# hjmkt/wrenc

Hardware: AMD Instinct MI355X
Metric: all-intra encode fps at fixed QP (CTU RD search + final pass); bit-exactness vs the CPU oracle is checked in `parity` (higher is better)
Workload: dtype u8/i16/i32 (+i64 trellis costs, f32 RD cost)

## Files before the change

wrenc_amd/csrc/dev_quant.h:

```cpp
#pragma once

namespace wrenc {

__device__ __forceinline__ long long ldq_at(Ctx c, int bits) {
    return bits < 256 ? (long long)SHT.ldq[bits] : c.k->ldq[bits];
}
__device__ __forceinline__ long long lv_at(Ctx c, int a) {
    return a < 256 ? (long long)SHT.lv[a] : c.k->lv[a];
}
template <int CTRL>
__device__ __forceinline__ int dpp_quad(int v) {
    return __builtin_amdgcn_mov_dpp(v, CTRL, 0xF, 0xF, true);
}

struct DecMasks {
    uint32_t m01, m23;
};
__device__ __forceinline__ DecMasks dec_masks(const uint16_t* dec16, int p) {
    const uint2 v = *(const uint2*)(dec16 + (p >> 4) * 4);
    DecMasks m;
    m.m01 = v.x;
    m.m23 = v.y;
    return m;
}
__device__ __forceinline__ int dec_nib(DecMasks m, int p) {
    const int k = p & 15;
    const uint32_t t01 = m.m01 >> k, t23 = m.m23 >> k;
    return (int)((t01 & 1u) | ((t01 >> 15) & 2u) | ((t23 & 1u) << 2) | ((t23 >> 13) & 8u));
}

constexpr int kMapId = 0x03020100;
__device__ __forceinline__ int compose_map(int g2, int g1) {
    return (int)__builtin_amdgcn_perm(0u, (uint32_t)g2, (uint32_t)g1);
}
__device__ __forceinline__ int position_map(int tc, int qd, bool dcn, int nib) {
    int pv = 0;
    if (tc != 0) {
        const int b0 = (qd >> 1) & 1;
        const int b1 = dcn ? b0 : (((qd + 1) >> 1) & 1);
        pv = nib ^ (b0 ? 3 : 0) ^ (b1 ? 12 : 0);
    }
    const unsigned x = (unsigned)(pv ^ 10);
    return (int)(0x01010000u + (((x * 0x00204081u) & 0x01010101u) << 1));
}

constexpr int kNoBranch = 1 << 27;

__device__ __forceinline__ int ldq_fast(const Ctx& c, int idx) {
    int v = SHT.ldq[min(idx, 255)];
    if (__ballot(idx > 255) != 0ULL) {
        if (idx > 255) v = (int)c.k->ldq[idx];
    }
    return v;
}

__device__ __forceinline__ int quotient(const CONST_AS DevConst* k, int tc, int sh, int off) {
    int S = (int)((unsigned)tc << sh) - off;
    if (tc < 0) S = -S;
    return tc == 0 ? 0 : (int)(__umulhi((unsigned)S, k->div_magic) >> k->div_shift);
}

__device__ __forceinline__ void chunk_entry(const Ctx& c, int* en, int tc, int qd, bool dcn, bool tzp, int sh, int off,
                                            int lsc, int ldq1, int* par0_out, int* par1_out, int* adj_out,
                                            int* ovf) {
    const bool nz = tc != 0;
    int c0d[2], c1d[2], par[2];
#pragma unroll
    for (int d = 0; d < 2; ++d) {
        const int a0 = (qd + (dcn ? 0 : d)) >> 1;
        const int a1 = a0 + 1;
        int q0 = (a0 > 0 || dcn) ? 2 * a0 - d : 0;
        int q1 = 2 * a1 - d;
        if (tc < 0) {
            q0 = -q0;
            q1 = -q1;
        }
        const int d0 = abs(tc - ((M24(q0, lsc) + off) >> sh));
        const int d1 = abs(tc - ((M24(q1, lsc) + off) >> sh));
        if (nz && a1 + 1 >= 1024) *ovf = 1;
        const int l0 = ldq_fast(c, min(a0 + 1, 1023)), l1 = ldq_fast(c, min(a1 + 1, 1023));
        c0d[d] = nz ? 128 * d0 + l0 : ldq1;
        c1d[d] = nz ? 128 * d1 + l1 : kNoBranch;
        par[d] = nz ? (a0 & 1) : 0;
    }
    const int a00 = qd >> 1;
    const bool zero0 = !nz || a00 == 0;
    const int c0tz = nz ? (a00 == 0 ? c0d[0] - ldq1 : c0d[0]) : 0;
    const int c0s0 = tzp ? c0tz : c0d[0];
    const int p0 = par[0], p1 = par[1];
    en[0] = 2 * (p0 ? c1d[0] : c0s0) + p0;
    en[1] = 2 * (p0 ? c0s0 : c1d[0]) + 1 - p0;
    en[2] = 2 * (p0 ? c1d[0] : c0d[0]) + p0;
    en[3] = 2 * (p0 ? c0d[0] : c1d[0]) + 1 - p0;
    en[4] = 2 * (p1 ? c1d[1] : c0d[1]) + p1;
    en[5] = 2 * (p1 ? c0d[1] : c1d[1]) + 1 - p1;
    *par0_out = p0;
    *par1_out = p1;
    *adj_out = (tzp && zero0) ? 1 : 0;
}

__device__ __forceinline__ int lv_fast(const Ctx& c, int a) {
    int v = SHT.lv[min(a, 255)];
    if (__ballot(a > 255) != 0ULL) {
        if (a > 255) v = (int)c.k->lv[a];
    }
    return v;
}

__device__ __forceinline__ int emit_level(const Ctx& c, int tc, int qd, bool dcn, int nib, int p, int j, int& state,
                                          unsigned& zmask, long long& sum_nz, int& fnz, int& ovf) {
    const int dl = state > 1 ? 1 : 0;
    const bool nz = tc != 0;
    const int a = nz ? ((qd + (dcn ? 0 : dl)) >> 1) + ((nib >> state) & 1) : 0;
    int q = (nz && (a > 0 || dcn)) ? 2 * a - dl : 0;
    if (tc < 0) q = -q;
    const int qc = abs(q);
    const bool zero = qc == 0;
    zmask |= (zero ? 1u : 0u) << j;
    const int aw = (qc + dl) >> 1;
    if (!zero && aw >= 1024) ovf = 1;
    const int lv = lv_fast(c, min(aw, 1023));
    sum_nz += zero ? 0 : lv;
    fnz = zero ? fnz : min(fnz, p);
    state = (0x7D28 >> (2 * (2 * state + (a & 1)))) & 3;
    return q;
}

__device__ __forceinline__ unsigned shift_in_less(unsigned bits, int kb, int ka) {
    return __builtin_amdgcn_alignbit(bits, (unsigned)(kb - ka), 31);
}

constexpr int kAlphaInf = 1 << 28;
struct HeadK {
    int ldq1, ldq2, ldq3;
    int dp1, dp2, dp3, dn1, dn2, dn3;
};
__device__ __forceinline__ HeadK head_consts(int sh, int off, int lsc) {
    HeadK h;
    h.ldq1 = uni(SHT.ldq[1]);
    h.ldq2 = uni(SHT.ldq[2]);
    h.ldq3 = uni(SHT.ldq[3]);
    h.dp1 = (lsc + off) >> sh;
    h.dp2 = (2 * lsc + off) >> sh;
    h.dp3 = (3 * lsc + off) >> sh;
    h.dn1 = (-lsc + off) >> sh;
    h.dn2 = (-2 * lsc + off) >> sh;
    h.dn3 = (-3 * lsc + off) >> sh;
    return h;
}
__device__ __forceinline__ int head_alpha(int tc, int qd, bool dcn, const HeadK& h, bool* bad) {
    const bool neg = tc < 0;
    const int d1 = abs(tc - (neg ? h.dn1 : h.dp1));
    const int d2 = abs(tc - (neg ? h.dn2 : h.dp2));
    const int d3 = abs(tc - (neg ? h.dn3 : h.dp3));
    const int d1o = abs(tc - (neg ? h.dp1 : h.dn1));
    const int c0tz = 128 * abs(tc);
    const int c0d0 = c0tz + h.ldq1;
    const int c1d0 = 128 * d2 + h.ldq2;
    const int c0d1 = dcn ? 128 * d1o + h.ldq1 : (qd ? 128 * d1 + h.ldq2 : c0d0);
    const int c1d1 = (qd && !dcn) ? 128 * d3 + h.ldq3 : 128 * d1 + h.ldq2;
    int alpha = c1d0 - c0tz;
    int beta = min(min(c0d0, c0d1), c1d1) - c0tz;
    if (tc == 0) {
        alpha = kAlphaInf;
        beta = h.ldq1;
    }
    *bad = qd >= 2 || alpha < 0 || beta < 0 || h.ldq1 < 0;
    return min(alpha, kAlphaInf);
}
struct HeadT {
    int tn, cnt, tnd, cntd, tnq, cntq;
};
__device__ __forceinline__ HeadT head_ranges(const CONST_AS DevConst* k, int lg) {
    const CONST_AS int32_t* r = k->head_rng[lg - 2];
    HeadT t;
    t.tn = r[0];
    t.cnt = r[1];
    t.tnd = r[2];
    t.cntd = r[3];
    t.tnq = r[4];
    t.cntq = r[5];
    return t;
}
__device__ __forceinline__ bool head_bad(int tc, bool dcn, const HeadT& t) {
    return (unsigned)(tc + (dcn ? t.tnd : t.tn)) >= (unsigned)(dcn ? t.cntd : t.cnt);
}
__device__ __forceinline__ bool head_sig(int tc, const HeadT& t) { return (unsigned)(tc + t.tnq) >= (unsigned)t.cntq; }
__device__ __forceinline__ int head_alpha1(int tc, const HeadK& h) {
    const int d2 = abs(tc - (tc < 0 ? h.dn2 : h.dp2));
    return tc == 0 ? kAlphaInf : min(128 * d2 + h.ldq2 - 128 * abs(tc), kAlphaInf);
}
__device__ __forceinline__ void head_batch(int tc, int p, int P, bool valid, const HeadK& h, const HeadT& t, bool& open, int& arun, int& sb) {
    if (!open) return;
    const int alpha = head_alpha1(tc, h);
    const unsigned long long B = __ballot(valid && head_bad(tc, p == P - 1, t));
    if (B == 0ULL) {
        if (valid) arun = min(arun, alpha);
    } else {
        const int fb = (int)__builtin_ctzll(B);
        sb = (p - LANE + fb) >> 4;
        if (valid && LANE < (fb & ~15)) arun = min(arun, alpha);
        open = false;
    }
}
__device__ __forceinline__ int head_sb(bool open, int sb, int nsb) { return open ? nsb : sb; }
__device__ __forceinline__ bool head_test(int C, int st, int amin) {
    const int c0 = dpp_quad<0x00>(C);
    int m = st == 0 ? 0x7FFFFFFF : C;
    m = min(m, dpp_quad<0xB1>(m));
    m = min(m, dpp_quad<0x4E>(m));
    return (m - c0) + 2 * amin >= 0;
}

template <int LG>
__device__ __forceinline__ void solo_gather(int blk, int16_t* tcs, const HeadK& hk, const HeadT& ht, int& nzl, int& first, bool& open,
                                            int& arun, int& sb) {
    constexpr int P = 1 << (2 * LG), NB = (P + 63) / 64, G = 4;
    const int lane = LANE;
    const int row = lane >> 4;
    const int in4 = blk * P + scan_nib_offset(LG, scan_nib(lane & 15));
#pragma unroll
    for (int g = 0; g < NB; g += G) {
        int tcb[G];
#pragma unroll
        for (int t = 0; t < G; ++t) {
            if (g + t >= NB) continue;
            const int p = 64 * (g + t) + lane;
            tcb[t] = p < P ? (int)SH.r1[scan_word_origin(scan_batch_word(LG, g + t), row) + in4] : 0;
        }
#pragma unroll
        for (int t = 0; t < G; ++t) {
            if (g + t >= NB) continue;
            const int p0 = 64 * (g + t), p = p0 + lane;
            const bool valid = p < P;
            const int tc = tcb[t];
            nzl |= tc;
            if (valid) tcs[blk * P + p] = (int16_t)tc;
            if (first == P) {
                const unsigned long long sig = __ballot(head_sig(tc, ht));
                if (sig != 0ULL) first = p0 + (int)__builtin_ctzll(sig);
            }
            head_batch(tc, p, P, valid, hk, ht, open, arun, sb);
        }
    }
}

__device__ __forceinline__ long long quantize_solo(Ctx c, int lg, int nb, int* overflow, bool* any_level) {
    c = uni(c);
    lg = uni(lg);
    nb = uni(nb);
    const CONST_AS DevConst* k = c.k;
    const int n = 1 << lg;
    const int P = n * n;
    const int lgP = 2 * lg;
    const int sh = 8 + lg - 5 + 1;
    const int off = (1 << sh) >> 1;
    const int lsc = k->lsc;
    int16_t* tcs = (int16_t*)SH.r2;
    int32_t* cc = (int32_t*)SH.r1;
    uint16_t* dec16 = (uint16_t*)SH.decw;
    PROF_MARK(q0_);
    *any_level = false;
#ifdef WRENC_EXP_SKIP_QUANT
    for (int i = LANE; i < (nb * P) / 8; i += 64) *(uint4*)&SH.r1[8 * i] = make_uint4(0u, 0u, 0u, 0u);
    WSYNC();
    return 0;
#endif
    const HeadK hk = head_consts(sh, off, lsc);
    const HeadT ht = head_ranges(k, lg);
    const int nsb = P >> 4;
    int istar0 = P, istar1 = P, sbs0 = nsb - 1, sbs1 = nsb - 1, amin0 = kAlphaInf, amin1 = kAlphaInf;
    int nzl = 0;
#pragma unroll 1
    for (int blk = 0; blk < nb; ++blk) {
        int first = P, arun = kAlphaInf, sb = nsb - 1;
        bool open = true;
        switch (lg) {
        case 2: solo_gather<2>(blk, tcs, hk, ht, nzl, first, open, arun, sb); break;
        case 3: solo_gather<3>(blk, tcs, hk, ht, nzl, first, open, arun, sb); break;
        case 4: solo_gather<4>(blk, tcs, hk, ht, nzl, first, open, arun, sb); break;
        default: solo_gather<5>(blk, tcs, hk, ht, nzl, first, open, arun, sb); break;
        }
        sb = head_sb(open, sb, nsb);
        if (sb > 0 && sb < nsb) arun = wave_min_i32(arun);
        if (blk) {
            istar1 = first;
            sbs1 = sb;
            amin1 = arun;
        } else {
            istar0 = first;
            sbs0 = sb;
            amin0 = arun;
        }
    }
    if (__ballot(nzl != 0) == 0ULL) return 0;
    WSYNC();
    if (sbs0 == nsb && (nb == 1 || sbs1 == nsb)) {
        for (int i = LANE; i < (nb * P) / 8; i += 64) *(uint4*)&SH.r1[8 * i] = make_uint4(0u, 0u, 0u, 0u);
        WSYNC();
        PROF_MARK(qz_);
        PROF_ADD2(PH_QPRE, q0_, qz_);
        return 0;
    }
    if (LANE < sbs0) *(uint2*)(dec16 + LANE * 4) = make_uint2(0u, 0u);
    if (nb == 2 && LANE < sbs1) *(uint2*)(dec16 + (P >> 2) + LANE * 4) = make_uint2(0u, 0u);
    PROF_MARK(q1_);
    PROF_ADD2(PH_QPRE, q0_, q1_);
    const int ldq1 = hk.ldq1;
    const int st = LANE & 3;
    const int CH = min(P, nb == 2 ? 32 : 64);
    const int quad = LANE >> 2;
    const bool walker = quad < nb;
    const int wblk = walker ? quad : 0;
    const int32_t* wcc = (const int32_t*)SH.r1 + wblk * CH * 6;
    const int cls = st == 0 ? 0 : (st == 1 ? 1 : 2);
    uint16_t* wdec = dec16 + wblk * (P >> 2);
    int wsb = wblk ? sbs1 : sbs0;
    const int wamin = wblk ? amin1 : amin0;
    int lowest = nb == 2 ? min(sbs0, sbs1) : sbs0;
    int C = 0;
    int ovf = 0;
    for (int base = P - CH; base >= 0 && base + CH > 16 * lowest; base -= CH) {
        PROF_MARK(qb0_);
        WSYNC();
        {
            const bool mine = LANE < nb * CH;
            const int blk = LANE >= CH ? 1 : 0;
            const int i = LANE - blk * CH;
            const int p = base + i;
            int par0 = 0, par1 = 0, adj = 0;
            if (mine) {
                const int tc = tcs[blk * P + p];
                chunk_entry(c, cc + LANE * 6, tc, quotient(k, tc, sh, off), p == P - 1, p <= (blk ? istar1 : istar0),
                            sh, off, lsc, ldq1, &par0, &par1, &adj, &ovf);
            }
            const unsigned long long b0 = __ballot(mine && par0), b1 = __ballot(mine && par1), ba = __ballot(mine && adj);
            if (mine && (LANE & 15) == 0) {
                uint16_t* pm = SH.q_pm[blk][i >> 4];
                pm[0] = (uint16_t)(b0 >> LANE);
                pm[1] = (uint16_t)(b1 >> LANE);
                pm[2] = (uint16_t)((ba >> (LANE + 15)) & 1);
            }
        }
        WSYNC();
        PROF_MARK(qb1_);
        if (walker) {
            for (int g16 = CH - 16; g16 >= 0; g16 -= 16) {
                const int sb = (base + g16) >> 4;
                if (sb < lowest) break;
                const uint16_t* pm = SH.q_pm[wblk][g16 >> 4];
                const unsigned parmask = pm[st > 1 ? 1 : 0];
                const bool adj = st == 0 && pm[2] != 0;
                int2 cur[16];
#pragma unroll
                for (int kk = 0; kk < 16; ++kk) cur[kk] = *(const int2*)&wcc[(g16 + kk) * 6 + 2 * cls];
                unsigned bits = 0;
#pragma unroll
                for (int kk = 15; kk >= 0; --kk) {
                    const int2 e = cur[kk];
                    const int KA = e.x + dpp_quad<0xD8>(C);
                    const int KB = e.y + dpp_quad<0x72>(C);
                    C = min(KA, KB) & ~1;
                    bits = shift_in_less(bits, KB, KA);
                    if (kk == 15) {
                        const bool choseB = KB < KA;
                        const bool pick1 = choseB != (((parmask >> 15) & 1) != 0);
                        if (!pick1 && adj) C -= 2 * ldq1;
                    }
                }
                bits ^= parmask;
                int m = min(C, dpp_quad<0xB1>(C));
                m = min(m, dpp_quad<0x4E>(m));
                C -= m;
                wdec[sb * 4 + st] = (uint16_t)bits;
                const bool proven = head_test(C, st, wamin);
                if (sb == wsb && sb > 0 && !proven) wsb = 0;
                lowest = __builtin_amdgcn_readlane(wsb, 0);
                if (nb == 2) lowest = min(lowest, __builtin_amdgcn_readlane(wsb, 4));
            }
        }
        lowest = __builtin_amdgcn_readlane(wsb, 0);
        if (nb == 2) lowest = min(lowest, __builtin_amdgcn_readlane(wsb, 4));
        PROF_MARK(qb3_);
        PROF_ADD2(PH_QB_PRE, qb0_, qb1_);
        PROF_ADD2(PH_QB_WALK, qb1_, qb3_);
    }
    WSYNC();
    PROF_MARK(q2_);
    PROF_ADD2(PH_QBACK, q1_, q2_);
    const int start0 = 16 * __builtin_amdgcn_readlane(wsb, 0), start1 = nb == 2 ? 16 * __builtin_amdgcn_readlane(wsb, 4) : 0;
    for (int i = LANE; i < (nb * P) / 8; i += 64) *(uint4*)&SH.r1[8 * i] = make_uint4(0u, 0u, 0u, 0u);
    WSYNC();
    const int half = nb == 2 ? 32 : 64;
    const int blk = nb == 2 ? (LANE >> 5) : 0;
    const int lane_in = LANE & (half - 1);
    const int start = blk ? start1 : start0;
    int per = 1;
    while (per * half < P - start) per *= 2;
    const int p0 = start + lane_in * per;
    const bool act = p0 < P;
    const int16_t* btcs = tcs + blk * P;
    const uint16_t* bdec = dec16 + blk * (P >> 2);
    int fmap = kMapId;
    const DecMasks dm = dec_masks(bdec, act ? p0 : 0);
    const int org = blk * P + scan_sb_origin(lg, act ? p0 >> 4 : 0);
    if (act) {
        for (int j = 0; j < per; ++j) {
            const int p = p0 + j;
            const int tc = btcs[p];
            fmap = compose_map(position_map(tc, quotient(k, tc, sh, off), p == P - 1, dec_nib(dm, p)), fmap);
        }
    }
    int pre = fmap;
    pre = compose_map(pre, __builtin_amdgcn_update_dpp(kMapId, pre, 0x111, 0xF, 0xF, false));
    pre = compose_map(pre, __builtin_amdgcn_update_dpp(kMapId, pre, 0x112, 0xF, 0xF, false));
    pre = compose_map(pre, __builtin_amdgcn_update_dpp(kMapId, pre, 0x114, 0xF, 0xF, false));
    pre = compose_map(pre, __builtin_amdgcn_update_dpp(kMapId, pre, 0x118, 0xF, 0xF, false));
    pre = compose_map(pre, __builtin_amdgcn_update_dpp(kMapId, pre, 0x142, 0xA, 0xF, false));
    if (nb == 1) pre = compose_map(pre, __builtin_amdgcn_update_dpp(kMapId, pre, 0x143, 0xC, 0xF, false));
    int entry = __builtin_amdgcn_update_dpp(0, pre, 0x138, 0xF, 0xF, false) & 3;
    if (lane_in == 0) entry = 0;
    long long sum_nz = 0;
    unsigned zmask = 0;
    int fnz = P;
    if (act) {
        int state = entry;
        unsigned long long nibs = scan_nibs_from(p0 & 15);
        for (int j = 0; j < per; ++j, nibs >>= 4) {
            const int p = p0 + j;
            const int tc = btcs[p];
            SH.r1[org + scan_nib_offset(lg, (int)nibs & 15)] = (int16_t)emit_level(c, tc, quotient(k, tc, sh, off), p == P - 1, dec_nib(dm, p), p, j,
                                                                                  state, zmask, sum_nz, fnz, ovf);
        }
    }
    const int pf = group_min_i32(fnz, half);
    if (act)
        sum_nz += (long long)__popc(zmask >> min(max(pf - p0 + 1, 0), 16)) * SHT.lv[0];
    *any_level = __ballot(pf < P) != 0ULL;
    const long long sum = wave_sum_i64(sum_nz);
    if (__ballot(ovf != 0) != 0ULL) *overflow = 1;
    WSYNC();
    PROF_MARK(q3_);
    PROF_ADD2(PH_QTRACE, q2_, q3_);
    return sum;
}

__device__ __forceinline__ int quantize_p16_reg(Ctx c, int nb, int coef, int* overflow, long long lvl[4], int* any_mask) {
    c = uni(c);
    nb = uni(nb);
    const int lane = lane_fresh();
    const CONST_AS DevConst* k = c.k;
    constexpr int P = 16, lg = 2;
    constexpr int sh = 8 + lg - 5 + 1;
    constexpr int off = (1 << sh) >> 1;
    const int lsc = k->lsc;
    int32_t* cc = (int32_t*)SH.r1;
    PROF_MARK(q0_);
    const int blk = lane >> 4, p = lane & 15;
    const bool mine = blk < nb;
#ifdef WRENC_EXP_SKIP_QUANT
    lvl[0] = lvl[1] = lvl[2] = lvl[3] = 0;
    *any_mask = 0;
    WSYNC();
    return 0;
#endif
    const HeadT ht = head_ranges(k, 2);
    const int at = 16 * blk + scan_nib(p);
    int tc = __builtin_amdgcn_ds_bpermute(4 * at, coef);
    if (!mine) tc = 0;
    const int istar = row_min_i32(head_sig(tc, ht) ? p : P);
    const unsigned long long nzb = __ballot(tc != 0);
    lvl[0] = lvl[1] = lvl[2] = lvl[3] = 0;
    *any_mask = 0;
    if (nzb == 0ULL) return 0;
    if (__ballot(mine && head_bad(tc, p == P - 1, ht)) == 0ULL) return 0;
    PROF_MARK(q1_);
    PROF_ADD2(PH_QPRE, q0_, q1_);
    WSYNC();
    const int qd = quotient(k, tc, sh, off);
    const int ldq1 = (int)ldq_at(c, 1);
    int ovf = 0;
    {
        int par0 = 0, par1 = 0, adj = 0;
        if (mine) chunk_entry(c, cc + lane * 6, tc, qd, p == P - 1, p <= istar, sh, off, lsc, ldq1, &par0, &par1, &adj, &ovf);
        const unsigned long long b0 = __ballot(mine && par0), b1 = __ballot(mine && par1), ba = __ballot(mine && adj);
        if (mine && p == 0) {
            uint16_t* pm = SH.q_pm[0][blk];
            pm[0] = (uint16_t)(b0 >> lane);
            pm[1] = (uint16_t)(b1 >> lane);
            pm[2] = (uint16_t)((ba >> (lane + 15)) & 1);
        }
    }
    WSYNC();
    PROF_MARK(qb1_);
    uint16_t* dec16 = (uint16_t*)SH.decw;
    {
        const int st = lane & 3, quad = lane >> 2;
        if (quad < nb) {
            const int cls = st == 0 ? 0 : (st == 1 ? 1 : 2);
            const int32_t* wcc = cc + quad * P * 6;
            const uint16_t* pm = SH.q_pm[0][quad];
            const unsigned parmask = pm[st > 1 ? 1 : 0];
            const bool adj = st == 0 && pm[2] != 0;
            int2 cur[16];
#pragma unroll
            for (int kk = 0; kk < 16; ++kk) cur[kk] = *(const int2*)&wcc[kk * 6 + 2 * cls];
            unsigned bits = 0;
            int C = 0;
#pragma unroll
            for (int kk = 15; kk >= 0; --kk) {
                const int2 e = cur[kk];
                const int KA = e.x + dpp_quad<0xD8>(C);
                const int KB = e.y + dpp_quad<0x72>(C);
                C = min(KA, KB) & ~1;
                bits = shift_in_less(bits, KB, KA);
                if (kk == 15) {
                    const bool choseB = KB < KA;
                    const bool pick1 = choseB != (((parmask >> 15) & 1) != 0);
                    if (!pick1 && adj) C -= 2 * ldq1;
                }
            }
            bits ^= parmask;
            dec16[quad * 4 + st] = (uint16_t)bits;
        }
    }
    WSYNC();
    PROF_MARK(q2_);
    PROF_ADD2(PH_QBACK, q1_, q2_);
    PROF_ADD2(PH_QB_WALK, qb1_, q2_);
    const DecMasks dm = dec_masks(dec16 + blk * 4, 0);
    const int nib = dec_nib(dm, p);
    int pre = mine ? position_map(tc, qd, p == P - 1, nib) : kMapId;
    pre = compose_map(pre, __builtin_amdgcn_update_dpp(kMapId, pre, 0x111, 0xF, 0xF, false));
    pre = compose_map(pre, __builtin_amdgcn_update_dpp(kMapId, pre, 0x112, 0xF, 0xF, false));
    pre = compose_map(pre, __builtin_amdgcn_update_dpp(kMapId, pre, 0x114, 0xF, 0xF, false));
    pre = compose_map(pre, __builtin_amdgcn_update_dpp(kMapId, pre, 0x118, 0xF, 0xF, false));
    int entry = __builtin_amdgcn_update_dpp(0, pre, 0x111, 0xF, 0xF, false) & 3;
    if (p == 0) entry = 0;
    long long sum_nz = 0;
    unsigned zmask = 0;
    int fnz = P;
    int level = 0;
    if (mine) {
        int state = entry;
        level = (int16_t)emit_level(c, tc, qd, p == P - 1, nib, p, 0, state, zmask, sum_nz, fnz, ovf);
    }
    level = __builtin_amdgcn_ds_permute(4 * at, level);
    const int pf = row_min_i32(fnz);
    if (mine && (zmask & 1u) && p > pf) sum_nz += SHT.lv[0];
    {
        const long long hi = sum_nz >> 24;
        const int ra = row_sum_i32((int)(sum_nz & 0xFFFFFF)), rb = row_sum_i32((int)(hi & 0xFFFFFF)), rc = row_sum_i32((int)(hi >> 24));
#pragma unroll
        for (int b = 0; b < 4; ++b) {
            const long long a0 = (long long)(unsigned)__builtin_amdgcn_readlane(ra, 16 * b);
            const long long a1 = (long long)(unsigned)__builtin_amdgcn_readlane(rb, 16 * b);
            const long long a2 = (long long)__builtin_amdgcn_readlane(rc, 16 * b);
            lvl[b] = a0 + ((a1 + (a2 << 24)) << 24);
            if (__builtin_amdgcn_readlane(pf, 16 * b) < P) *any_mask |= 1 << b;
        }
    }
    if (__ballot(ovf != 0) != 0ULL) *overflow = 1;
    WSYNC();
    PROF_MARK(q3_);
    PROF_ADD2(PH_QTRACE, q2_, q3_);
    return level;
}
__device__ __forceinline__ int dequantize4_lane(const Ctx& c, int level) {
    constexpr int sh = 8 + 2 - 5 + 1, off = (1 << sh) >> 1;
    const int v = (M24(level, c.k->lsc) + off) >> sh;
    return min(max(v, -32768), 32767);
}


__device__ __forceinline__ void trace_rows64(const Ctx& c, int nblk, const int16_t* tcs, const uint16_t* dec16, int rbase,
                                             int sh, int off, long long lvl[4], bool any[4], int& ovf, int start = 0) {
    const int lane = lane_fresh();
    const int row = lane >> 4, i16 = lane & 15;
    const CONST_AS DevConst* k = c.k;
    const int per = start >= 48 ? 1 : (start >= 32 ? 2 : 4);
    const int p0 = start + i16 * per;
    const bool act = row < nblk && p0 < 64;
    const int b = row < nblk ? row : 0;
    const int16_t* btcs = tcs + b * 64;
    const DecMasks dm = dec_masks(dec16 + b * 16, act ? p0 : 0);
    const int org = rbase + b * 64 + scan_sb_origin_ct<3>(act ? p0 >> 4 : 0);
    int fmap = kMapId;
    if (act) {
        for (int j = 0; j < per; ++j) {
            const int p = p0 + j;
            const int tc = btcs[p];
            fmap = compose_map(position_map(tc, quotient(k, tc, sh, off), p == 63, dec_nib(dm, p)), fmap);
        }
    }
    int pre = fmap;
    pre = compose_map(pre, __builtin_amdgcn_update_dpp(kMapId, pre, 0x111, 0xF, 0xF, false));
    pre = compose_map(pre, __builtin_amdgcn_update_dpp(kMapId, pre, 0x112, 0xF, 0xF, false));
    pre = compose_map(pre, __builtin_amdgcn_update_dpp(kMapId, pre, 0x114, 0xF, 0xF, false));
    pre = compose_map(pre, __builtin_amdgcn_update_dpp(kMapId, pre, 0x118, 0xF, 0xF, false));
    int entry = __builtin_amdgcn_update_dpp(0, pre, 0x111, 0xF, 0xF, false) & 3;
    if (i16 == 0) entry = 0;
    long long sum_nz = 0;
    unsigned zmask = 0;
    int fnz = 64;
    if (act) {
        int state = entry;
        unsigned long long nibs = scan_nibs_from(p0 & 15);
        for (int j = 0; j < per; ++j, nibs >>= 4) {
            const int p = p0 + j;
            const int tc = btcs[p];
            SH.r1[org + scan_nib_offset(3, (int)nibs & 15)] = (int16_t)emit_level(c, tc, quotient(k, tc, sh, off), p == 63, dec_nib(dm, p), p, j,
                                                                                 state, zmask, sum_nz, fnz, ovf);
        }
    }
    const int pf = row_min_i32(fnz);
    if (act) sum_nz += (long long)__popc(zmask >> min(max(pf - p0 + 1, 0), 16)) * SHT.lv[0];
    const long long hi = sum_nz >> 24;
    const int ra = row_sum_i32((int)(sum_nz & 0xFFFFFF)), rb = row_sum_i32((int)(hi & 0xFFFFFF)), rc = row_sum_i32((int)(hi >> 24));
#pragma unroll
    for (int bb = 0; bb < 4; ++bb) {
        const long long a0 = (long long)(unsigned)__builtin_amdgcn_readlane(ra, 16 * bb);
        const long long a1 = (long long)(unsigned)__builtin_amdgcn_readlane(rb, 16 * bb);
        const long long a2 = (long long)__builtin_amdgcn_readlane(rc, 16 * bb);
        lvl[bb] = a0 + ((a1 + (a2 << 24)) << 24);
        any[bb] = __builtin_amdgcn_readlane(pf, 16 * bb) < 64;
    }
}

__device__ __forceinline__ void trace_rows16(const Ctx& c, int nblk, const int16_t* tcs, const uint16_t* dec16, int rbase,
                                             int sh, int off, long long lvl[4], bool any[4], int& ovf) {
    const int lane = lane_fresh();
    const int row = lane >> 4, i16 = lane & 15;
    const CONST_AS DevConst* k = c.k;
    const bool mine = row < nblk;
    const int bb = mine ? row : 0;
    const int tc = mine ? (int)tcs[bb * 16 + i16] : 0;
    const int qd = quotient(k, tc, sh, off);
    const DecMasks dm = dec_masks(dec16 + bb * 4, 0);
    const int nib = dec_nib(dm, i16);
    int pre = mine ? position_map(tc, qd, i16 == 15, nib) : kMapId;
    pre = compose_map(pre, __builtin_amdgcn_update_dpp(kMapId, pre, 0x111, 0xF, 0xF, false));
    pre = compose_map(pre, __builtin_amdgcn_update_dpp(kMapId, pre, 0x112, 0xF, 0xF, false));
    pre = compose_map(pre, __builtin_amdgcn_update_dpp(kMapId, pre, 0x114, 0xF, 0xF, false));
    pre = compose_map(pre, __builtin_amdgcn_update_dpp(kMapId, pre, 0x118, 0xF, 0xF, false));
    int entry = __builtin_amdgcn_update_dpp(0, pre, 0x111, 0xF, 0xF, false) & 3;
    if (i16 == 0) entry = 0;
    long long sum_nz = 0;
    unsigned zmask = 0;
    int fnz = 16;
    if (mine) {
        int state = entry;
        SH.r1[rbase + bb * 16 + scan_nib(i16)] = (int16_t)emit_level(c, tc, qd, i16 == 15, nib, i16, 0, state, zmask, sum_nz, fnz, ovf);
    }
    const int pf = row_min_i32(fnz);
    if (mine && (zmask & 1u) && i16 > pf) sum_nz += SHT.lv[0];
    const long long hi = sum_nz >> 24;
    const int ra = row_sum_i32((int)(sum_nz & 0xFFFFFF)), rb = row_sum_i32((int)(hi & 0xFFFFFF)), rc = row_sum_i32((int)(hi >> 24));
#pragma unroll
    for (int b = 0; b < 4; ++b) {
        const long long a0 = (long long)(unsigned)__builtin_amdgcn_readlane(ra, 16 * b);
        const long long a1 = (long long)(unsigned)__builtin_amdgcn_readlane(rb, 16 * b);
        const long long a2 = (long long)__builtin_amdgcn_readlane(rc, 16 * b);
        lvl[b] = a0 + ((a1 + (a2 << 24)) << 24);
        any[b] = __builtin_amdgcn_readlane(pf, 16 * b) < 16;
    }
}

__device__ __forceinline__ void trace_wave256(const Ctx& c, const int16_t* tcs, const uint16_t* dec16, int rbase,
                                              int sh, int off, long long* lvl, bool* any, int& ovf, int start = 0) {
    const int lane = lane_fresh();
    const CONST_AS DevConst* k = c.k;
    const int per = start >= 192 ? 1 : (start >= 128 ? 2 : 4);
    const int p0 = start + lane * per;
    const bool act = p0 < 256;
    const DecMasks dm = dec_masks(dec16, act ? p0 : 0);
    const int org = rbase + scan_sb_origin_ct<4>(act ? p0 >> 4 : 0);
    int fmap = kMapId;
    if (act) {
        for (int j = 0; j < per; ++j) {
            const int p = p0 + j;
            const int tc = tcs[p];
            fmap = compose_map(position_map(tc, quotient(k, tc, sh, off), p == 255, dec_nib(dm, p)), fmap);
        }
    }
    int pre = fmap;
    pre = compose_map(pre, __builtin_amdgcn_update_dpp(kMapId, pre, 0x111, 0xF, 0xF, false));
    pre = compose_map(pre, __builtin_amdgcn_update_dpp(kMapId, pre, 0x112, 0xF, 0xF, false));
    pre = compose_map(pre, __builtin_amdgcn_update_dpp(kMapId, pre, 0x114, 0xF, 0xF, false));
    pre = compose_map(pre, __builtin_amdgcn_update_dpp(kMapId, pre, 0x118, 0xF, 0xF, false));
    pre = compose_map(pre, __builtin_amdgcn_update_dpp(kMapId, pre, 0x142, 0xA, 0xF, false));
    pre = compose_map(pre, __builtin_amdgcn_update_dpp(kMapId, pre, 0x143, 0xC, 0xF, false));
    int entry = __builtin_amdgcn_update_dpp(0, pre, 0x138, 0xF, 0xF, false) & 3;
    if (lane == 0) entry = 0;
    long long sum_nz = 0;
    unsigned zmask = 0;
    int fnz = 256;
    if (act) {
        int state = entry;
        unsigned long long nibs = scan_nibs_from(p0 & 15);
        for (int j = 0; j < per; ++j, nibs >>= 4) {
            const int p = p0 + j;
            const int tc = tcs[p];
            SH.r1[org + scan_nib_offset(4, (int)nibs & 15)] = (int16_t)emit_level(c, tc, quotient(k, tc, sh, off), p == 255, dec_nib(dm, p), p, j,
                                                                                 state, zmask, sum_nz, fnz, ovf);
        }
    }
    const int pf = wave_min_i32(fnz);
    if (act) sum_nz += (long long)__popc(zmask >> min(max(pf - p0 + 1, 0), 16)) * SHT.lv[0];
    *any = pf < 256;
    *lvl = wave_sum_i64(sum_nz);
}

template <int LGL>
__device__ __forceinline__ void quantize_pk(Ctx c, int nc, int* overflow, long long lvl_y[3], long long lvl_c[3], bool* any_y,
                                            bool* any_c) {
    static_assert(LGL == 3 || LGL == 4, "8x8 and 16x16 CUs");
    c = uni(c);
    nc = uni(nc);
    const int lane = lane_fresh();
    const CONST_AS DevConst* k = c.k;
    constexpr int PL = 1 << (2 * LGL), PC = PL / 4;
    constexpr int SBL = PL / 16, SBC = PC / 16;
    constexpr int shl = 8 + LGL - 5 + 1, offl = (1 << shl) >> 1;
    constexpr int shc = shl - 1, offc = (1 << shc) >> 1;
    const int lsc = k->lsc;
    int16_t* tcs = (int16_t*)SH.r2;
    int32_t* cc = (int32_t*)SH.r1;
    uint16_t* dec16 = (uint16_t*)SH.decw;
    uint16_t* ist = &SH.q_pm[1][0][0];
    const int row = lane >> 4, i16 = lane & 15;
    const int nL = PL * nc;
    const int nch = 2 * nc;
    PROF_MARK(q0_);
    lvl_y[0] = lvl_y[1] = lvl_y[2] = 0;
    lvl_c[0] = lvl_c[1] = lvl_c[2] = 0;
    *any_y = false;
    *any_c = false;
#ifdef WRENC_EXP_SKIP_QUANT
    for (int i = lane; i < (nL + nch * PC) / 8; i += 64) *(uint4*)&SH.r1[8 * i] = make_uint4(0u, 0u, 0u, 0u);
    WSYNC();
    return;
#endif
    int nzl = 0;
    int v_low = 0, v_amin = kAlphaInf;
    const HeadK hkl = head_consts(shl, offl, lsc);
    const HeadT htl = head_ranges(k, LGL), htc = head_ranges(k, LGL - 1);
    const int nib = scan_nib(i16);
#pragma unroll 1
    for (int cd = 0; cd < nc; ++cd) {
        int first = PL, arun = kAlphaInf, sb = SBL - 1;
        bool open = true;
#pragma unroll
        for (int t = 0; t < PL / 64; ++t) {
            const int p = lane + 64 * t;
            const int tc = SH.r1[cd * PL + scan_word_origin(scan_batch_word(LGL, t), row) + scan_nib_offset(LGL, nib)];
            nzl |= tc;
            tcs[cd * PL + p] = (int16_t)tc;
            if (first == PL) {
                const unsigned long long sig = __ballot(head_sig(tc, htl));
                if (sig != 0ULL) first = (p - lane) + (int)__builtin_ctzll(sig);
            }
            head_batch(tc, p, PL, true, hkl, htl, open, arun, sb);
        }
        sb = head_sb(open, sb, SBL);
        if (sb > 0 && sb < SBL) arun = wave_min_i32(arun);
        if (lane == 0) ist[cd] = (uint16_t)first;
        if (lane == cd) {
            v_low = sb;
            v_amin = arun;
        }
    }
    if constexpr (LGL == 3) {
#pragma unroll
        for (int ps = 0; ps < 2; ++ps) {
            const int blk = 4 * ps + row;
            const bool mine = blk < nch;
            int tc = 0;
            if (mine) {
                tc = SH.r1[nL + blk * 16 + nib];
                nzl |= tc;
                tcs[nL + blk * 16 + i16] = (int16_t)tc;
            }
            const int first = row_min_i32(head_sig(tc, htc) ? i16 : 16);
            if (mine && i16 == 0) ist[4 + blk] = (uint16_t)first;
            const unsigned long long B = __ballot(mine && head_bad(tc, i16 == 15, htc));
#pragma unroll
            for (int rw = 0; rw < 4; ++rw)
                if (lane == 4 + 4 * ps + rw) v_low = (((B >> (16 * rw)) & 0xFFFFULL) == 0ULL) ? 1 : 0;
        }
    } else {
        const HeadK hkc = head_consts(shc, offc, lsc);
#pragma unroll 1
        for (int b = 0; b < nch; ++b) {
            const int tc = SH.r1[nL + b * PC + scan_word_origin(scan_batch_word(LGL - 1, 0), row) + scan_nib_offset(LGL - 1, nib)];
            nzl |= tc;
            tcs[nL + b * PC + lane] = (int16_t)tc;
            const unsigned long long sig = __ballot(head_sig(tc, htc));
            const int first = sig != 0ULL ? (int)__builtin_ctzll(sig) : PC;
            int arun = kAlphaInf, sb = SBC - 1;
            bool open = true;
            head_batch(tc, lane, PC, true, hkc, htc, open, arun, sb);
            sb = head_sb(open, sb, SBC);
            if (sb > 0 && sb < SBC) arun = wave_min_i32(arun);
            if (lane == 0) ist[4 + b] = (uint16_t)first;
            if (lane == 4 + b) {
                v_low = sb;
                v_amin = arun;
            }
        }
    }
    if (__ballot(nzl != 0) == 0ULL) return;
    {
        const bool todo = lane < 12 && (lane < nc || (lane >= 4 && lane < 4 + nch)) && v_low < (lane < 4 ? SBL : SBC);
        if (__ballot(todo) == 0ULL) {
            WSYNC();
            for (int i = lane; i < (nL + nch * PC) / 8; i += 64) *(uint4*)&SH.r1[8 * i] = make_uint4(0u, 0u, 0u, 0u);
            WSYNC();
            PROF_MARK(qz_);
            PROF_ADD2(PH_QPRE, q0_, qz_);
            return;
        }
    }
    {
        constexpr int kMaxNc = LGL == 3 ? 3 : 2;
        constexpr int kDecWords = (4 * SBL * kMaxNc + 4 * SBC * 2 * kMaxNc + 3) / 4;
        static_assert(kDecWords <= 64 && 8 * kDecWords <= 512, "decw");
        if (lane < (4 * SBL * nc + 4 * SBC * nch + 3) / 4) *(uint2*)(dec16 + 4 * lane) = make_uint2(0u, 0u);
    }
    WSYNC();
    PROF_MARK(q1_);
    PROF_ADD2(PH_QPRE, q0_, q1_);
    const int ldq1 = (int)ldq_at(c, 1);
    const int st = lane & 3, quad = lane >> 2;
    const int cls = st == 0 ? 0 : (st == 1 ? 1 : 2);
    int C = 0;
    int ovf = 0;
    int rid[4] = {-1, -1, -1, -1}, rleft[4] = {0, 0, 0, 0}, rlow[4] = {0, 0, 0, 0}, ramin[4] = {0, 0, 0, 0};
    int next_chain = 0;
    const int nct = nc + nch;
#pragma unroll 1
    for (;;) {
        bool fresh[4];
        bool any_row = false;
#pragma unroll
        for (int j = 0; j < 4; ++j) {
            fresh[j] = false;
            if (rleft[j] == 0) {
                rid[j] = -1;
                while (next_chain < nct) {
                    const int id = next_chain < nc ? next_chain : 4 + (next_chain - nc);
                    ++next_chain;
                    const int low = __builtin_amdgcn_readlane(v_low, id);
                    const int len = (id < 4 ? SBL : SBC) - low;
                    if (len <= 0) continue;
                    rid[j] = id;
                    rlow[j] = low;
                    ramin[j] = __builtin_amdgcn_readlane(v_amin, id);
                    rleft[j] = len;
                    fresh[j] = true;
                    break;
                }
            }
            any_row = any_row || rid[j] >= 0;
        }
        if (!any_row) break;
        const int myid = row == 0 ? rid[0] : (row == 1 ? rid[1] : (row == 2 ? rid[2] : rid[3]));
        const int mysb = (row == 0 ? rlow[0] + rleft[0] : (row == 1 ? rlow[1] + rleft[1] : (row == 2 ? rlow[2] + rleft[2] : rlow[3] + rleft[3]))) - 1;
        {
            const bool mine = myid >= 0;
            const bool is_l = myid < 4;
            const int p = 16 * mysb + i16;
            const int sh = is_l ? shl : shc, off = is_l ? offl : offc;
            int par0 = 0, par1 = 0, adj = 0;
            if (mine) {
                const int tc = tcs[is_l ? myid * PL + p : nL + (myid - 4) * PC + p];
                const int first = ist[myid];
                chunk_entry(c, cc + lane * 6, tc, quotient(k, tc, sh, off), p == (is_l ? PL - 1 : PC - 1), p <= first, sh, off, lsc, ldq1,
                            &par0, &par1, &adj, &ovf);
            }
            const unsigned long long b0 = __ballot(mine && par0), b1 = __ballot(mine && par1), ba = __ballot(mine && adj);
            if (mine && i16 == 0) {
                uint16_t* pm = SH.q_pm[0][row];
                pm[0] = (uint16_t)(b0 >> lane);
                pm[1] = (uint16_t)(b1 >> lane);
                pm[2] = (uint16_t)((ba >> (lane + 15)) & 1);
            }
        }
        WSYNC();
        PROF_MARK(qb1_);
        bool unproven = false;
        if (quad < 4) {
            const int wid = quad == 0 ? rid[0] : (quad == 1 ? rid[1] : (quad == 2 ? rid[2] : rid[3]));
            const int wleft = quad == 0 ? rleft[0] : (quad == 1 ? rleft[1] : (quad == 2 ? rleft[2] : rleft[3]));
            const int wlow = quad == 0 ? rlow[0] : (quad == 1 ? rlow[1] : (quad == 2 ? rlow[2] : rlow[3]));
            const int wamin = quad == 0 ? ramin[0] : (quad == 1 ? ramin[1] : (quad == 2 ? ramin[2] : ramin[3]));
            const bool wfresh = quad == 0 ? fresh[0] : (quad == 1 ? fresh[1] : (quad == 2 ? fresh[2] : fresh[3]));
            if (wid >= 0) {
                if (wfresh) C = 0;
                const int wsb = wlow + wleft - 1;
                const int32_t* wcc = cc + quad * 16 * 6;
                const uint16_t* pm = SH.q_pm[0][quad];
                const unsigned parmask = pm[st > 1 ? 1 : 0];
                const bool adj = st == 0 && pm[2] != 0;
                int2 cur[16];
#pragma unroll
                for (int kk = 0; kk < 16; ++kk) cur[kk] = *(const int2*)&wcc[kk * 6 + 2 * cls];
                unsigned bits = 0;
#pragma unroll
                for (int kk = 15; kk >= 0; --kk) {
                    const int2 e = cur[kk];
                    const int KA = e.x + dpp_quad<0xD8>(C);
                    const int KB = e.y + dpp_quad<0x72>(C);
                    C = min(KA, KB) & ~1;
                    bits = shift_in_less(bits, KB, KA);
                    if (kk == 15) {
                        const bool choseB = KB < KA;
                        const bool pick1 = choseB != (((parmask >> 15) & 1) != 0);
                        if (!pick1 && adj) C -= 2 * ldq1;
                    }
                }
                bits ^= parmask;
                int m = min(C, dpp_quad<0xB1>(C));
                m = min(m, dpp_quad<0x4E>(m));
                C -= m;
                dec16[(wid < 4 ? 4 * SBL * wid : 4 * SBL * nc + 4 * SBC * (wid - 4)) + 4 * wsb + st] = (uint16_t)bits;
                const bool proven = head_test(C, st, wamin);
                unproven = wleft == 1 && wlow > 0 && !proven;
            }
        }
        const unsigned long long ub = __ballot(unproven);
        WSYNC();
        PROF_MARK(qb2_);
        PROF_ADD2(PH_QB_WALK, qb1_, qb2_);
#pragma unroll
        for (int j = 0; j < 4; ++j)
            if (rid[j] >= 0) {
                --rleft[j];
                if ((ub >> (4 * j)) & 1ULL) {
                    rleft[j] = rlow[j];
                    rlow[j] = 0;
                    if (lane == rid[j]) v_low = 0;
                }
            }
    }
    PROF_MARK(q2_);
    PROF_ADD2(PH_QBACK, q1_, q2_);
    for (int i = lane; i < (nL + nch * PC) / 8; i += 64) *(uint4*)&SH.r1[8 * i] = make_uint4(0u, 0u, 0u, 0u);
    WSYNC();
    const unsigned live = (unsigned)__ballot(lane < 12 && (lane < nc || (lane >= 4 && lane < 4 + nch)) && v_low < (lane < 4 ? SBL : SBC));
    PROF_CNT(PH_SPARSE + 0, 1);
    int n_with = 0;
    if constexpr (LGL == 3) {
        long long l4[4];
        bool a4[4];
        PROF_CNT(PH_SPARSE + 1, 1);
        PROF_CNT(PH_SPARSE + 2, (live & 0x7u) == 0);
        const int s0_ = 16 * __builtin_amdgcn_readlane(v_low, 0), s1_ = 16 * __builtin_amdgcn_readlane(v_low, 1),
                  s2_ = 16 * __builtin_amdgcn_readlane(v_low, 2);
        trace_rows64(c, nc, tcs, dec16, 0, shl, offl, l4, a4, ovf, row == 0 ? s0_ : (row == 1 ? s1_ : (row == 2 ? s2_ : 0)));
#pragma unroll
        for (int b = 0; b < 3; ++b)
            if (b < nc) {
                lvl_y[b] = l4[b];
                if (a4[b]) *any_y = true;
                n_with += a4[b];
            }
        PROF_CNT(PH_SPARSE + 9, n_with != 0);
        PROF_CNT(PH_SPARSE + 10, n_with ? nc - n_with : 0);
#pragma unroll
        for (int ps = 0; ps < 2; ++ps) {
            if (4 * ps >= nch) continue;
            PROF_CNT(PH_SPARSE + 3, 1);
            if (!(live & (0xF0u << (4 * ps)))) {
                PROF_CNT(PH_SPARSE + 4, 1);
                continue;
            }
            trace_rows16(c, min(4, nch - 4 * ps), tcs + nL + 64 * ps, dec16 + 4 * SBL * nc + 16 * ps, nL + 64 * ps, shc, offc, l4, a4, ovf);
#pragma unroll
            for (int b = 0; b < 4; ++b)
                if (4 * ps + b < nch) {
                    lvl_c[(4 * ps + b) >> 1] += l4[b];
                    if (a4[b]) *any_c = true;
                }
        }
    } else {
#pragma unroll 1
        for (int cd = 0; cd < nc; ++cd) {
            long long l1;
            bool a1;
            PROF_CNT(PH_SPARSE + 5, 1);
            PROF_CNT(PH_SPARSE + 6, ((live >> cd) & 1u) == 0);
            trace_wave256(c, tcs + cd * PL, dec16 + 4 * SBL * cd, cd * PL, shl, offl, &l1, &a1, ovf,
                          16 * __builtin_amdgcn_readlane(v_low, cd));
            if (cd == 0)
                lvl_y[0] = l1;
            else
                lvl_y[1] = l1;
            if (a1) *any_y = true;
            n_with += a1;
        }
        PROF_CNT(PH_SPARSE + 11, n_with != 0);
        PROF_CNT(PH_SPARSE + 12, n_with ? nc - n_with : 0);
        PROF_CNT(PH_SPARSE + 7, 1);
        if (live & 0xF0u) {
            long long l4[4];
            bool a4[4];
            const int s4_ = 16 * __builtin_amdgcn_readlane(v_low, 4), s5_ = 16 * __builtin_amdgcn_readlane(v_low, 5),
                      s6_ = 16 * __builtin_amdgcn_readlane(v_low, 6), s7_ = 16 * __builtin_amdgcn_readlane(v_low, 7);
            trace_rows64(c, nch, tcs + nL, dec16 + 4 * SBL * nc, nL, shc, offc, l4, a4, ovf,
                         row == 0 ? s4_ : (row == 1 ? s5_ : (row == 2 ? s6_ : s7_)));
            n_with = 0;
#pragma unroll
            for (int b = 0; b < 4; ++b)
                if (b < nch) {
                    lvl_c[b >> 1] += l4[b];
                    if (a4[b]) *any_c = true;
                    n_with += a4[b];
                }
            PROF_CNT(PH_SPARSE + 13, n_with != 0);
            PROF_CNT(PH_SPARSE + 14, n_with ? nch - n_with : 0);
        } else {
            PROF_CNT(PH_SPARSE + 8, 1);
        }
    }
    (void)n_with;
    if (__ballot(ovf != 0) != 0ULL) *overflow = 1;
    WSYNC();
    PROF_MARK(q3_);
    PROF_ADD2(PH_QTRACE, q2_, q3_);
}

__device__ __forceinline__ void dequantize_t(Ctx c, int lg, int nb, int o1 = 0) {
    c = uni(c);
    lg = uni(lg);
    nb = uni(nb);
    o1 = uni(o1);
    const int n = 1 << lg;
    const int nn = n * n;
    const int sh = 8 + lg - 5 + 1;
    const int off = (1 << sh) >> 1;
    const int lsc = c.k->lsc;
    int16_t* out = (int16_t*)SH.r2;
    for (int i = LANE; i < nb * nn; i += 64) {
        const int blk = i >> (2 * lg), ii = i & (nn - 1);
        const int x = ii & (n - 1), y = ii >> lg;
        int v = (M24(SH.r1[o1 + i], lsc) + off) >> sh;
        v = min(max(v, -32768), 32767);
        out[blk * nn + x * n + y] = (int16_t)v;
    }
    WSYNC();
}

}
```

Baseline: 261.0.

## Keep parity masks in registers, share ldq lookups, cache traceback inputs

The per-chunk parity and adjacency ballots now stay in wave-uniform registers. The walkers extract their 16-bit masks by shifting, which replaces a round trip through the shared q_pm array. chunk_entry loads three consecutive ldq table entries once and picks among them, instead of four separate ballot-guarded lookups. The final-pass loops are unrolled to at most four positions and cache tc, quotient and nibble, so the second emit loop no longer reloads and recomputes them. This adds register pressure and a wave-uniform switch between the unrolled and generic paths.

```diff
diff --git a/wrenc_amd/csrc/dev_quant.h b/wrenc_amd/csrc/dev_quant.h
--- a/wrenc_amd/csrc/dev_quant.h
+++ b/wrenc_amd/csrc/dev_quant.h
@@ -46,18 +46,19 @@
 
 constexpr int kNoBranch = 1 << 27;
 
-__device__ __forceinline__ int ldq_fast(const Ctx& c, int idx) {
-    int v = SHT.ldq[min(idx, 255)];
-    if (__ballot(idx > 255) != 0ULL) {
-        if (idx > 255) v = (int)c.k->ldq[idx];
-    }
-    return v;
-}
-
 __device__ __forceinline__ int quotient(const CONST_AS DevConst* k, int tc, int sh, int off) {
     int S = (int)((unsigned)tc << sh) - off;
     if (tc < 0) S = -S;
     return tc == 0 ? 0 : (int)(__umulhi((unsigned)S, k->div_magic) >> k->div_shift);
+}
+
+struct TracePos {
+    int tc[4], qd[4], nib[4];
+};
+__device__ __forceinline__ void trace_pos_load(TracePos& t, int j, const CONST_AS DevConst* k, int tc, int sh, int off, DecMasks dm, int p) {
+    t.tc[j] = tc;
+    t.qd[j] = quotient(k, tc, sh, off);
+    t.nib[j] = dec_nib(dm, p);
 }
 
 __device__ __forceinline__ void chunk_entry(const Ctx& c, int* en, int tc, int qd, bool dcn, bool tzp, int sh, int off,
@@ -65,6 +66,17 @@
                                             int* ovf) {
     const bool nz = tc != 0;
     int c0d[2], c1d[2], par[2];
+    const int a = qd >> 1;
+    const int e = (!dcn && (qd & 1)) ? 1 : 0;
+    const int32_t* tq = &SHT.ldq[min(a, 252)];
+    int t1 = tq[1], t2 = tq[2], t3 = tq[3];
+    if (__ballot(a > 252) != 0ULL) {
+        if (a > 252) {
+            t1 = (int)ldq_at(c, min(a + 1, 1023));
+            t2 = (int)ldq_at(c, min(a + 2, 1023));
+            t3 = (int)ldq_at(c, min(a + 3, 1023));
+        }
+    }
 #pragma unroll
     for (int d = 0; d < 2; ++d) {
         const int a0 = (qd + (dcn ? 0 : d)) >> 1;
@@ -78,7 +90,7 @@
         const int d0 = abs(tc - ((M24(q0, lsc) + off) >> sh));
         const int d1 = abs(tc - ((M24(q1, lsc) + off) >> sh));
         if (nz && a1 + 1 >= 1024) *ovf = 1;
-        const int l0 = ldq_fast(c, min(a0 + 1, 1023)), l1 = ldq_fast(c, min(a1 + 1, 1023));
+        const int l0 = (d && e) ? t2 : t1, l1 = (d && e) ? t3 : t2;
         c0d[d] = nz ? 128 * d0 + l0 : ldq1;
         c1d[d] = nz ? 128 * d1 + l1 : kNoBranch;
         par[d] = nz ? (a0 & 1) : 0;
@@ -323,6 +335,7 @@
     for (int base = P - CH; base >= 0 && base + CH > 16 * lowest; base -= CH) {
         PROF_MARK(qb0_);
         WSYNC();
+        unsigned long long b0, b1, ba;
         {
             const bool mine = LANE < nb * CH;
             const int blk = LANE >= CH ? 1 : 0;
@@ -334,13 +347,9 @@
                 chunk_entry(c, cc + LANE * 6, tc, quotient(k, tc, sh, off), p == P - 1, p <= (blk ? istar1 : istar0),
                             sh, off, lsc, ldq1, &par0, &par1, &adj, &ovf);
             }
-            const unsigned long long b0 = __ballot(mine && par0), b1 = __ballot(mine && par1), ba = __ballot(mine && adj);
-            if (mine && (LANE & 15) == 0) {
-                uint16_t* pm = SH.q_pm[blk][i >> 4];
-                pm[0] = (uint16_t)(b0 >> LANE);
-                pm[1] = (uint16_t)(b1 >> LANE);
-                pm[2] = (uint16_t)((ba >> (LANE + 15)) & 1);
-            }
+            b0 = __ballot(mine && par0);
+            b1 = __ballot(mine && par1);
+            ba = __ballot(mine && adj);
         }
         WSYNC();
         PROF_MARK(qb1_);
@@ -348,9 +357,9 @@
             for (int g16 = CH - 16; g16 >= 0; g16 -= 16) {
                 const int sb = (base + g16) >> 4;
                 if (sb < lowest) break;
-                const uint16_t* pm = SH.q_pm[wblk][g16 >> 4];
-                const unsigned parmask = pm[st > 1 ? 1 : 0];
-                const bool adj = st == 0 && pm[2] != 0;
+                const int at = wblk * CH + g16;
+                const unsigned parmask = (uint16_t)((st > 1 ? b1 : b0) >> at);
+                const bool adj = st == 0 && ((ba >> (at + 15)) & 1ULL) != 0ULL;
                 int2 cur[16];
 #pragma unroll
                 for (int kk = 0; kk < 16; ++kk) cur[kk] = *(const int2*)&wcc[(g16 + kk) * 6 + 2 * cls];
@@ -404,7 +413,17 @@
     int fmap = kMapId;
     const DecMasks dm = dec_masks(bdec, act ? p0 : 0);
     const int org = blk * P + scan_sb_origin(lg, act ? p0 >> 4 : 0);
-    if (act) {
+    const bool few = __ballot(per > 4) == 0ULL;
+    TracePos tp;
+    if (few) {
+#pragma unroll
+        for (int j = 0; j < 4; ++j) {
+            if (!(act && j < per)) continue;
+            const int p = p0 + j;
+            trace_pos_load(tp, j, k, btcs[p], sh, off, dm, p);
+            fmap = compose_map(position_map(tp.tc[j], tp.qd[j], p == P - 1, tp.nib[j]), fmap);
+        }
+    } else if (act) {
         for (int j = 0; j < per; ++j) {
             const int p = p0 + j;
             const int tc = btcs[p];
@@ -423,7 +442,16 @@
     long long sum_nz = 0;
     unsigned zmask = 0;
     int fnz = P;
-    if (act) {
+    if (few) {
+        int state = entry;
+        const unsigned long long nibs = scan_nibs_from(p0 & 15);
+#pragma unroll
+        for (int j = 0; j < 4; ++j) {
+            if (!(act && j < per)) continue;
+            SH.r1[org + scan_nib_offset(lg, (int)(nibs >> (4 * j)) & 15)] =
+                (int16_t)emit_level(c, tp.tc[j], tp.qd[j], p0 + j == P - 1, tp.nib[j], p0 + j, j, state, zmask, sum_nz, fnz, ovf);
+        }
+    } else if (act) {
         int state = entry;
         unsigned long long nibs = scan_nibs_from(p0 & 15);
         for (int j = 0; j < per; ++j, nibs >>= 4) {
@@ -480,16 +508,13 @@
     const int qd = quotient(k, tc, sh, off);
     const int ldq1 = (int)ldq_at(c, 1);
     int ovf = 0;
+    unsigned long long b0, b1, ba;
     {
         int par0 = 0, par1 = 0, adj = 0;
         if (mine) chunk_entry(c, cc + lane * 6, tc, qd, p == P - 1, p <= istar, sh, off, lsc, ldq1, &par0, &par1, &adj, &ovf);
-        const unsigned long long b0 = __ballot(mine && par0), b1 = __ballot(mine && par1), ba = __ballot(mine && adj);
-        if (mine && p == 0) {
-            uint16_t* pm = SH.q_pm[0][blk];
-            pm[0] = (uint16_t)(b0 >> lane);
-            pm[1] = (uint16_t)(b1 >> lane);
-            pm[2] = (uint16_t)((ba >> (lane + 15)) & 1);
-        }
+        b0 = __ballot(mine && par0);
+        b1 = __ballot(mine && par1);
+        ba = __ballot(mine && adj);
     }
     WSYNC();
     PROF_MARK(qb1_);
@@ -499,9 +524,8 @@
         if (quad < nb) {
             const int cls = st == 0 ? 0 : (st == 1 ? 1 : 2);
             const int32_t* wcc = cc + quad * P * 6;
-            const uint16_t* pm = SH.q_pm[0][quad];
-            const unsigned parmask = pm[st > 1 ? 1 : 0];
-            const bool adj = st == 0 && pm[2] != 0;
+            const unsigned parmask = (uint16_t)((st > 1 ? b1 : b0) >> (16 * quad));
+            const bool adj = st == 0 && ((ba >> (16 * quad + 15)) & 1ULL) != 0ULL;
             int2 cur[16];
 #pragma unroll
             for (int kk = 0; kk < 16; ++kk) cur[kk] = *(const int2*)&wcc[kk * 6 + 2 * cls];
@@ -586,12 +610,13 @@
     const DecMasks dm = dec_masks(dec16 + b * 16, act ? p0 : 0);
     const int org = rbase + b * 64 + scan_sb_origin_ct<3>(act ? p0 >> 4 : 0);
     int fmap = kMapId;
-    if (act) {
-        for (int j = 0; j < per; ++j) {
-            const int p = p0 + j;
-            const int tc = btcs[p];
-            fmap = compose_map(position_map(tc, quotient(k, tc, sh, off), p == 63, dec_nib(dm, p)), fmap);
-        }
+    TracePos tp;
+#pragma unroll
+    for (int j = 0; j < 4; ++j) {
+        if (!(act && j < per)) continue;
+        const int p = p0 + j;
+        trace_pos_load(tp, j, k, btcs[p], sh, off, dm, p);
+        fmap = compose_map(position_map(tp.tc[j], tp.qd[j], p == 63, tp.nib[j]), fmap);
     }
     int pre = fmap;
     pre = compose_map(pre, __builtin_amdgcn_update_dpp(kMapId, pre, 0x111, 0xF, 0xF, false));
@@ -603,14 +628,14 @@
     long long sum_nz = 0;
     unsigned zmask = 0;
     int fnz = 64;
-    if (act) {
+    {
         int state = entry;
-        unsigned long long nibs = scan_nibs_from(p0 & 15);
-        for (int j = 0; j < per; ++j, nibs >>= 4) {
-            const int p = p0 + j;
-            const int tc = btcs[p];
-            SH.r1[org + scan_nib_offset(3, (int)nibs & 15)] = (int16_t)emit_level(c, tc, quotient(k, tc, sh, off), p == 63, dec_nib(dm, p), p, j,
-                                                                                 state, zmask, sum_nz, fnz, ovf);
+        const unsigned long long nibs = scan_nibs_from(p0 & 15);
+#pragma unroll
+        for (int j = 0; j < 4; ++j) {
+            if (!(act && j < per)) continue;
+            SH.r1[org + scan_nib_offset(3, (int)(nibs >> (4 * j)) & 15)] =
+                (int16_t)emit_level(c, tp.tc[j], tp.qd[j], p0 + j == 63, tp.nib[j], p0 + j, j, state, zmask, sum_nz, fnz, ovf);
         }
     }
     const int pf = row_min_i32(fnz);
@@ -676,12 +701,13 @@
     const DecMasks dm = dec_masks(dec16, act ? p0 : 0);
     const int org = rbase + scan_sb_origin_ct<4>(act ? p0 >> 4 : 0);
     int fmap = kMapId;
-    if (act) {
-        for (int j = 0; j < per; ++j) {
-            const int p = p0 + j;
-            const int tc = tcs[p];
-            fmap = compose_map(position_map(tc, quotient(k, tc, sh, off), p == 255, dec_nib(dm, p)), fmap);
-        }
+    TracePos tp;
+#pragma unroll
+    for (int j = 0; j < 4; ++j) {
+        if (!(act && j < per)) continue;
+        const int p = p0 + j;
+        trace_pos_load(tp, j, k, tcs[p], sh, off, dm, p);
+        fmap = compose_map(position_map(tp.tc[j], tp.qd[j], p == 255, tp.nib[j]), fmap);
     }
     int pre = fmap;
     pre = compose_map(pre, __builtin_amdgcn_update_dpp(kMapId, pre, 0x111, 0xF, 0xF, false));
@@ -695,14 +721,14 @@
     long long sum_nz = 0;
     unsigned zmask = 0;
     int fnz = 256;
-    if (act) {
+    {
         int state = entry;
-        unsigned long long nibs = scan_nibs_from(p0 & 15);
-        for (int j = 0; j < per; ++j, nibs >>= 4) {
-            const int p = p0 + j;
-            const int tc = tcs[p];
-            SH.r1[org + scan_nib_offset(4, (int)nibs & 15)] = (int16_t)emit_level(c, tc, quotient(k, tc, sh, off), p == 255, dec_nib(dm, p), p, j,
-                                                                                 state, zmask, sum_nz, fnz, ovf);
+        const unsigned long long nibs = scan_nibs_from(p0 & 15);
+#pragma unroll
+        for (int j = 0; j < 4; ++j) {
+            if (!(act && j < per)) continue;
+            SH.r1[org + scan_nib_offset(4, (int)(nibs >> (4 * j)) & 15)] =
+                (int16_t)emit_level(c, tp.tc[j], tp.qd[j], p0 + j == 255, tp.nib[j], p0 + j, j, state, zmask, sum_nz, fnz, ovf);
         }
     }
     const int pf = wave_min_i32(fnz);
@@ -866,6 +892,7 @@
         if (!any_row) break;
         const int myid = row == 0 ? rid[0] : (row == 1 ? rid[1] : (row == 2 ? rid[2] : rid[3]));
         const int mysb = (row == 0 ? rlow[0] + rleft[0] : (row == 1 ? rlow[1] + rleft[1] : (row == 2 ? rlow[2] + rleft[2] : rlow[3] + rleft[3]))) - 1;
+        unsigned long long b0, b1, ba;
         {
             const bool mine = myid >= 0;
             const bool is_l = myid < 4;
@@ -878,13 +905,9 @@
                 chunk_entry(c, cc + lane * 6, tc, quotient(k, tc, sh, off), p == (is_l ? PL - 1 : PC - 1), p <= first, sh, off, lsc, ldq1,
                             &par0, &par1, &adj, &ovf);
             }
-            const unsigned long long b0 = __ballot(mine && par0), b1 = __ballot(mine && par1), ba = __ballot(mine && adj);
-            if (mine && i16 == 0) {
-                uint16_t* pm = SH.q_pm[0][row];
-                pm[0] = (uint16_t)(b0 >> lane);
-                pm[1] = (uint16_t)(b1 >> lane);
-                pm[2] = (uint16_t)((ba >> (lane + 15)) & 1);
-            }
+            b0 = __ballot(mine && par0);
+            b1 = __ballot(mine && par1);
+            ba = __ballot(mine && adj);
         }
         WSYNC();
         PROF_MARK(qb1_);
@@ -899,9 +922,8 @@
                 if (wfresh) C = 0;
                 const int wsb = wlow + wleft - 1;
                 const int32_t* wcc = cc + quad * 16 * 6;
-                const uint16_t* pm = SH.q_pm[0][quad];
-                const unsigned parmask = pm[st > 1 ? 1 : 0];
-                const bool adj = st == 0 && pm[2] != 0;
+                const unsigned parmask = (uint16_t)((st > 1 ? b1 : b0) >> (16 * quad));
+                const bool adj = st == 0 && ((ba >> (16 * quad + 15)) & 1ULL) != 0ULL;
                 int2 cur[16];
 #pragma unroll
                 for (int kk = 0; kk < 16; ++kk) cur[kk] = *(const int2*)&wcc[kk * 6 + 2 * cls];
```

Result: faster. 265.7, median of 6 (+1.8%).
